# secondlaw-ai/skyrim

Hardware: AMD Instinct MI355X
Metric: 6-h forecast steps/sec on 721x1440 state, 1/2/4/8 MI355X; per-channel max rel-err vs ref (higher is better)
Workload: dtype f16; 1 GPU; Pangu 6-h autoregressive rollout, 721x1440x69 state (13 levels x 5 vars + 4 surface), random-init weights (64 M params), state resident in HBM, 1 ensemble membe; parallelism=single GPU, members=1, finite=True, rounding=compensated, term_plan=0x66f

## Files before the change

### skyrim_amd/csrc/api.hip

```cpp
#include <cstdio>
#include <cstdlib>
#include <cstring>
#include <string>
#include <type_traits>
#include <vector>

#include "../../include/skyrim_pangu.h"
#include "launchers.h"

using namespace skp;

namespace {

constexpr int kDepths[4] = {2, 6, 6, 2};
constexpr int kBiasRows = 3312;

int pad_to(int n, int mult, int* front, int pad_mode) {
    const int padded = (n + mult - 1) / mult * mult;
    if (front) *front = pad_mode == SKPANGU_PAD_CENTRE ? (padded - n) / 2 : 0;
    return padded;
}

bool make_geom(const skpangu_config& c, Geom& g) {
    if (c.n_lat < 8 || c.n_lon <= 0 || c.n_lon % 96 != 0) return false;
// ... 165 lines not shown
                                   : (qa_fused(1) ? kDepths[1] : 0) + (qa_fused(2) ? kDepths[2] : 0);
            if (nqa > 0) {
                const double qa_fl = fl[C_ATTN0 + o] + fl[C_QKV0 + o];
                const double qa_by = nt * C * 2 + mw * C * sa + 3 * C * C * wb + (double)g.types[r] * heads * 3456 * 2;
                fl[C_ATTN0 + o] = nqa == nblk ? qa_fl : (nqa * qa_fl + (nblk - nqa) * fl[C_ATTN0 + o]) / nblk;
                by[C_ATTN0 + o] = nqa == nblk ? qa_by : (nqa * qa_by + (nblk - nqa) * by[C_ATTN0 + o]) / nblk;
            }
            if (fused_block) {
                fl[C_FC1_0 + o] = 4 * nt * C * 4 * C;  by[C_FC1_0 + o] = 2 * nt * C * 4 + 8 * C * C * wb;
                fl[C_FC1_0 + o] += 2 * mw * C * C;     by[C_FC1_0 + o] += nt * C * sa + C * C * wb;
            }
        }
        fl[C_EMBED] = 2 * hw * 112 * 192 + 2 * 7 * hw * 160 * 192; by[C_EMBED] = (69.0 + 3) * g.n_lat * g.n_lon * 4 + g.ntok[0] * 192.0 * 4;
        fl[C_DOWN] = 2.0 * g.ntok[1] * 768 * 384;                   by[C_DOWN] = g.ntok[0] * 192.0 * 4 + g.ntok[1] * 384.0 * 4;
        fl[C_UP] = 2.0 * g.ntok[1] * 384 * 768 + 2.0 * g.ntok[0] * 192 * 192;
        by[C_UP] = g.ntok[1] * 384.0 * 4 + 2 * g.ntok[0] * 192.0 * sa + g.ntok[0] * 192.0 * 4;
        fl[C_RECOVER] = 2 * hw * 384 * 64 + 2 * 7 * hw * 384 * 160; by[C_RECOVER] = 2 * g.ntok[0] * 192.0 * 4 + 69.0 * g.n_lat * g.n_lon * 4;
        int k = 0;
        for (int c = 0; c < C_COUNT && k < cap; ++c, ++k) {
            std::memset(&out[k], 0, sizeof(out[k]));
            std::strncpy(out[k].name, names[c], sizeof(out[k].name) - 1);
            out[k].launches = cnt[c]; out[k].total_ms = ms[c]; out[k].flops = fl[c]; out[k].bytes = by[c];
        }
        *n = k;
        prof_used = 0;
        return hipSuccess;
    }

    LinW<T> take_lin(Arena& a, int N, int ldd) {
        LinW<T> l;
        const long long plane = (long long)N * ldd;
// ... 50 lines not shown
        Arena a{base, 0};
        const size_t n0 = (size_t)g.ntok[0] * 192, n1 = (size_t)g.ntok[1] * 384;
        wk.xs_plane[0] = (long long)n0; wk.xs_plane[1] = (long long)n1;
        wk.X1s = a.take<T>(n0 * 2); wk.X2s = a.take<T>(n1 * 2); wk.X4s = a.take<T>(n0 * 2);
        const size_t m0 = (size_t)g.mwin[0] * 192, m1 = (size_t)g.mwin[1] * 384;
        q_elems = m0 > m1 ? m0 : m1;
        wk.qkv_plane = (long long)q_elems;
        wk.q = a.take<f16>(q_elems); wk.k = a.take<f16>(q_elems); wk.vt = a.take<f16>(q_elems);
        ao_elems = q_elems;
        wk.ao_plane = (long long)ao_elems;
        wk.ao = a.take<T>(ao_elems * NPL);
        const size_t h0 = (size_t)g.ntok[0] * 768, h1 = (size_t)g.ntok[1] * 1536;
        hid_elems = h0 > h1 ? h0 : h1;
        wk.hid_plane = (long long)hid_elems;
        wk.hid = a.take<T>(hid_elems * NPL);
        wk.u_plane = (long long)n0;
        wk.u = a.take<T>(n0 * NPL);
        wk.stats = a.take<float2>((size_t)g.ntok[1]);
        ws_bytes = (a.off + 255) / 256 * 256;
    }

    explicit Engine(const Geom& geom, int qkv_a1 = 0, int mlp_mode = 0, int term_plan = 0) : g(geom) {
        fused_qa = getenv("SKP_SPLIT_ATTN") == nullptr;
        fused_block = mlp_mode == 0;
        rt_qkv = (std::is_same<P, PrecF16x3>::value && qkv_a1 && mlp_mode == 0);
        plan2 = (std::is_same<P, PrecF16x3>::value && fused_block) ? term_plan : 0;
        wk.qkv_a1 = qkv_a1;
        params = build_params(g, nullptr);
        plan_prepared(nullptr);
        plan_workspace(nullptr);
    }
    size_t prepared_bytes() const override { return prep_bytes; }
// ... 249 lines not shown
        for (int i = 0; i < kDepths[3]; ++i) CK(block_planes(3, i, wk.X4s, s));
        mark(C_RECOVER, s);
        CK((op_recover<P>(g, w, wk.X1s, wk.X4s, out, wk, s)));
        mark(-1, s);
        return hipSuccess;
    }
#undef CK

    bool debug(const std::string& n, void** p, size_t* bytes) override {
        auto set = [&](const void* ptr, size_t b) { *p = const_cast<void*>(ptr); *bytes = b; return true; };
        if (n == "q") return set(wk.q, q_elems * sizeof(f16));
        if (n == "k") return set(wk.k, q_elems * sizeof(f16));
        if (n == "vt") return set(wk.vt, q_elems * sizeof(f16));
        if (n == "ao") return set(wk.ao, ao_elems * NPL * sizeof(T));
        if (n == "hid") return set(wk.hid, hid_elems * NPL * sizeof(T));
        if (n == "u") return set(wk.u, (size_t)g.ntok[0] * 192 * NPL * sizeof(T));
        if (n == "x1") return set(wk.X1s, (size_t)g.ntok[0] * 192 * 2 * sizeof(T));
        if (n == "x2") return set(wk.X2s, (size_t)g.ntok[1] * 384 * 2 * sizeof(T));
        if (n == "x4") return set(wk.X4s, (size_t)g.ntok[0] * 192 * 2 * sizeof(T));
        if (n.rfind("widx", 0) == 0 && n.size() == 6) {
            const int r = n[4] - '0', roll = n[5] - '0';
            if (r < 0 || r > 1 || roll < 0 || roll > 1) return false;
            return set(w.widx[r][roll], (size_t)g.mwin[r] * 4);
        }
        if (n.rfind("bias_exp", 0) == 0) {
            const int b = atoi(n.c_str() + 8);
            if (b < 0 || b > 15) return false;
            return set(w.blk[b].bias_cmp, bias_elems[b] * sizeof(f16));
        }
        return false;
    }
// ... 147 lines not shown
```

### skyrim_amd/csrc/epilogues.h

```cpp
#pragma once
#include "common.h"

namespace skp {

__device__ __forceinline__ void pin(f32x4& v) { asm volatile("" : "+v"(v)); }

__device__ __forceinline__ void add8(f32x4& lo, f32x4& hi, const float4& b0, const float4& b1) {
    lo[0] += b0.x; lo[1] += b0.y; lo[2] += b0.z; lo[3] += b0.w;
    hi[0] += b1.x; hi[1] += b1.y; hi[2] += b1.z; hi[3] += b1.w;
}

constexpr int kEpiReduceBytes = 4096;
constexpr int kEpiTableBytes = 8192;
constexpr int kEpiScratch = kEpiReduceBytes + kEpiTableBytes;


template <class T>
struct EpStorePlanes {
    static constexpr bool kDualOrder = false;
    template <class TC> __device__ __forceinline__ void init(char*, int, int) const {}
    const float* bias;
    int ld, row_off;
    T* out;
    long long plane;
    template <class TC, bool SWAP>
    __device__ __forceinline__ void run(f32x4 (&acc)[TC::FM][TC::FN], int m0w, int n0w, int lane, int, int, char*, int M, int N, int) const {
        static_assert(SWAP && TC::FN % 2 == 0, "swapped order, fragment pairs");
        const int lm = lane & 15, l8 = (lane >> 4) * 8;
#pragma unroll
        for (int bp = 0; bp < TC::FN / 2; ++bp) {
            const int n = n0w + bp * 32 + l8;
            const float* bsrc = bias + (n < N ? n : 0);
            const float4 b0 = (bias != nullptr) ? *reinterpret_cast<const float4*>(bsrc) : make_float4(0.f, 0.f, 0.f, 0.f);
            const float4 b1 = (bias != nullptr) ? *reinterpret_cast<const float4*>(bsrc + 4) : make_float4(0.f, 0.f, 0.f, 0.f);
#pragma unroll
            for (int a = 0; a < TC::FM; ++a) { add8(acc[a][2 * bp], acc[a][2 * bp + 1], b0, b1); pin(acc[a][2 * bp]); pin(acc[a][2 * bp + 1]); }
        }
#pragma unroll
        for (int a = 0; a < TC::FM; ++a) {
            const int m = m0w + a * 16 + lm;
            if (m >= M) continue;
#pragma unroll
            for (int bp = 0; bp < TC::FN / 2; ++bp) {
                const int n = n0w + bp * 32 + l8;
                if (n >= N) continue;
                const f32x4 &x = acc[a][2 * bp], &y = acc[a][2 * bp + 1];
                const float vv[8] = {x[0], x[1], x[2], x[3], y[0], y[1], y[2], y[3]};
                store8_planes<T, 2>(out + blk_off(m + row_off, n, ld), plane, vv);
            }
        }
    }
};

template <class T, int NPL>
struct EpGelu {
    static constexpr bool kDualOrder = false;
    template <class TC> __device__ __forceinline__ void init(char*, int, int) const {}
    T* out;
    long long plane;
    const float* bias;
    int ld;
    template <class TC, bool SWAP>
    __device__ __forceinline__ void run(f32x4 (&acc)[TC::FM][TC::FN], int m0w, int n0w, int lane, int, int, char*, int M, int N, int) const {
        static_assert(SWAP && TC::FN % 2 == 0, "swapped order, fragment pairs");
        const int lm = lane & 15, l8 = (lane >> 4) * 8;
// ... 127 lines not shown
                            old.b.x + y[4], old.b.y + y[5], old.b.z + y[6], old.b.w + y[7]};
        store8_planes<T, 2>(xs + blk_off(row, c, ld), plane, v);
    }
};
template <class T, int NPL>
struct SinkStore {
    T* out;
    long long plane;
    static constexpr bool kLoads = false;
    __device__ __forceinline__ f32x8 load(long long, int, int) const { return f32x8{}; }
    __device__ __forceinline__ void put(long long row, int ld, int c, const float (&y)[8], const f32x8&) const {
        store8_planes<T, NPL>(out + blk_off(row, c, ld), plane, y);
    }
};

template <class RowMap, class Sink, int GROUP = 1>
struct EpLayerNorm {
    static constexpr bool kDualOrder = false;
    template <class TC> __device__ __forceinline__ void init(char* tab, int tid, int n0) const {
        float* t = reinterpret_cast<float*>(tab);
        for (int i = tid; i < TC::BN; i += TC::THREADS) {
            t[i] = gamma[i];
            t[TC::BN + i] = beta[i];
            t[2 * TC::BN + i] = bias != nullptr ? bias[n0 + i] : 0.f;
        }
    }
    RowMap map;
    Sink sink;
    const float* bias;
    const float* gamma;
    const float* beta;
    float eps;
    int n_groups = 0;
    template <class TC, bool SWAP>
    __device__ __forceinline__ void run(f32x4 (&acc)[TC::FM][TC::FN], int m0w, int n0w, int lane, int wm, int wn, char* smem, int M, int N, int ntile) const {
        static_assert(SWAP && TC::FN % 2 == 0, "swapped order, fragment pairs");
        static_assert(GROUP == 1 || (GROUP == TC::FM && !Sink::kLoads), "grouped rows: one member per fragment, no residual");
        constexpr int FM = TC::FM, FN = TC::FN, FP = TC::FN / 2, WN = TC::WN, BM = TC::BM, BN = TC::BN;
        const int l15 = lane & 15, l8 = (lane >> 4) * 8;
        const int nloc0 = n0w - ntile * BN;
        float* red = reinterpret_cast<float*>(smem);
        const float* tab = reinterpret_cast<const float*>(smem + kEpiReduceBytes);
        static_assert(3 * BN * 4 <= kEpiTableBytes && 2 * BM * WN * 4 <= kEpiReduceBytes, "epilogue LDS scratch");
#pragma unroll
        for (int bp = 0; bp < FP; ++bp) {
            const float* bsrc = tab + 2 * BN + nloc0 + bp * 32 + l8;
            const float4 b0 = *reinterpret_cast<const float4*>(bsrc), b1 = *reinterpret_cast<const float4*>(bsrc + 4);
#pragma unroll
            for (int a = 0; a < FM; ++a) add8(acc[a][2 * bp], acc[a][2 * bp + 1], b0, b1);
        }
        long long drow[FM];
        bool ok[FM];
#pragma unroll
        for (int a = 0; a < FM; ++a) {
            const int m = m0w + a * 16 + l15;
            const long long r = map.dest(m < M ? m : 0, ntile);
            ok[a] = m < M && r >= 0;
            drow[a] = ok[a] ? r : 0;
        }
        constexpr int PRE = FM < 3 ? FM : 3;
        f32x8 old[Sink::kLoads ? FM : 1][Sink::kLoads ? FP : 1];
        if constexpr (Sink::kLoads) {
#pragma unroll
            for (int a = 0; a < PRE; ++a)
#pragma unroll
                for (int bp = 0; bp < FP; ++bp) old[a][bp] = sink.load(drow[a], BN, nloc0 + bp * 32 + l8);
        }
        float mean[FM], rstd[FM];
#pragma unroll
        for (int a = 0; a < FM; ++a) {
            float s = 0.f;
#pragma unroll
            for (int b = 0; b < FN; ++b) s += (acc[a][b][0] + acc[a][b][1]) + (acc[a][b][2] + acc[a][b][3]);
            s += __shfl_xor(s, 16);
            s += __shfl_xor(s, 32);
            if (lane < 16) red[(wm * TC::WTM + a * 16 + lane) * WN + wn] = s;
        }
        __syncthreads();
#pragma unroll
        for (int a = 0; a < FM; ++a) {
            float s = 0.f;
#pragma unroll
            for (int w = 0; w < WN; ++w) s += red[(wm * TC::WTM + a * 16 + l15) * WN + w];
            mean[a] = s * (1.0f / BN);
        }
        float* red2 = red + BM * WN;
#pragma unroll
        for (int a = 0; a < FM; ++a) {
            float s = 0.f;
#pragma unroll
            for (int b = 0; b < FN; ++b) {
#pragma unroll
                for (int r = 0; r < 4; ++r) { const float d = acc[a][b][r] - mean[a]; s += d * d; }
            }
            s += __shfl_xor(s, 16);
            s += __shfl_xor(s, 32);
            if (lane < 16) red2[(wm * TC::WTM + a * 16 + lane) * WN + wn] = s;
        }
        __syncthreads();
#pragma unroll
        for (int a = 0; a < FM; ++a) {
            float s = 0.f;
#pragma unroll
            for (int w = 0; w < WN; ++w) s += red2[(wm * TC::WTM + a * 16 + l15) * WN + w];
            rstd[a] = rsqrtf(s * (1.0f / BN) + eps);
        }
        if constexpr (GROUP > 1) {
            const long long grow = (long long)(m0w / (16 * FM)) * 16 + l15;
#pragma unroll
            for (int bp = 0; bp < FP; ++bp) {
                const int c = nloc0 + bp * 32 + l8;
                const float4 g0 = *reinterpret_cast<const float4*>(tab + c), g1 = *reinterpret_cast<const float4*>(tab + c + 4);
                const float4 e0 = *reinterpret_cast<const float4*>(tab + BN + c), e1 = *reinterpret_cast<const float4*>(tab + BN + c + 4);
                float y[8] = {0.f, 0.f, 0.f, 0.f, 0.f, 0.f, 0.f, 0.f};
#pragma unroll
                for (int a = 0; a < FM; ++a) {
                    const f32x4 &x = acc[a][2 * bp], &z = acc[a][2 * bp + 1];
                    const float mu = mean[a], rs = rstd[a];
                    y[0] += (x[0] - mu) * rs * g0.x + e0.x; y[1] += (x[1] - mu) * rs * g0.y + e0.y;
                    y[2] += (x[2] - mu) * rs * g0.z + e0.z; y[3] += (x[3] - mu) * rs * g0.w + e0.w;
                    y[4] += (z[0] - mu) * rs * g1.x + e1.x; y[5] += (z[1] - mu) * rs * g1.y + e1.y;
                    y[6] += (z[2] - mu) * rs * g1.z + e1.z; y[7] += (z[3] - mu) * rs * g1.w + e1.w;
                }
                if (grow < n_groups) sink.put(grow, BN, c, y, old[0][0]);
            }
            return;
        }
#pragma unroll
        for (int a = 0; a < FM; ++a) {
#pragma unroll
            for (int bp = 0; bp < FP; ++bp) {
                const int c = nloc0 + bp * 32 + l8;
                const float4 g0 = *reinterpret_cast<const float4*>(tab + c), g1 = *reinterpret_cast<const float4*>(tab + c + 4);
                const float4 e0 = *reinterpret_cast<const float4*>(tab + BN + c), e1 = *reinterpret_cast<const float4*>(tab + BN + c + 4);
                const f32x4 &x = acc[a][2 * bp], &z = acc[a][2 * bp + 1];
                const float mu = mean[a], rs = rstd[a];
                const float y[8] = {(x[0] - mu) * rs * g0.x + e0.x, (x[1] - mu) * rs * g0.y + e0.y, (x[2] - mu) * rs * g0.z + e0.z, (x[3] - mu) * rs * g0.w + e0.w,
                                    (z[0] - mu) * rs * g1.x + e1.x, (z[1] - mu) * rs * g1.y + e1.y, (z[2] - mu) * rs * g1.z + e1.z, (z[3] - mu) * rs * g1.w + e1.w};
                if (ok[a]) sink.put(drow[a], BN, c, y, Sink::kLoads ? old[a][bp] : old[0][0]);
            }
            if constexpr (Sink::kLoads) {
                if (a + PRE < FM) {
#pragma unroll
                    for (int bp = 0; bp < FP; ++bp) old[a + PRE][bp] = sink.load(drow[a + PRE], BN, nloc0 + bp * 32 + l8);
                }
            }
        }
    }
};

struct EpRecover {
    static constexpr bool kDualOrder = false;
    template <class TC> __device__ __forceinline__ void init(char* tab, int tid, int) const {
// ... 47 lines not shown
```

### skyrim_amd/csrc/gemm.h

```cpp
#pragma once
#include "common.h"
#include "epilogues.h"

namespace skp {

template <int BM_, int BN_, int BK_, int WM_, int WN_>
struct TileCfg {
    static constexpr int BM = BM_, BN = BN_, BK = BK_, WM = WM_, WN = WN_;
    static constexpr int THREADS = 64 * WM * WN;
    static constexpr int WTM = BM / WM, WTN = BN / WN;
    static constexpr int FM = WTM / 16, FN = WTN / 16;
    static constexpr int CPR = BK / 8;
    static constexpr int A_CHUNKS = (BM * CPR + THREADS - 1) / THREADS;
    static constexpr int W_CHUNKS = (BN * CPR + THREADS - 1) / THREADS;
    static_assert(WTM % 16 == 0 && WTN % 16 == 0, "wave tile must be a multiple of 16x16");
    static_assert(THREADS % CPR == 0, "thread->slot mapping");
    static_assert(BK == 32 || BK == 64, "BK");
};

template <class P, class AL, class EP>
struct GemmArgs {
    AL al;
    EP ep;
    const typename P::T* W;
// ... 162 lines not shown

template <class P, class TC, class AL, class EP>
inline hipError_t launch_gemm(const GemmArgs<P, AL, EP>& g, hipStream_t stream) {
    dim3 grid((g.N + TC::BN - 1) / TC::BN, (g.M + TC::BM - 1) / TC::BM);
    if (grid.x == 0 || grid.y == 0) return hipSuccess;
    constexpr int smem = gemm_smem_bytes<P, TC>() + kEpiScratch;
    static_assert(smem <= 160 * 1024, "LDS per block");
    if (smem > 64 * 1024) {
        hipError_t e = hipFuncSetAttribute(reinterpret_cast<const void*>(gemm_kernel<P, TC, AL, EP>), hipFuncAttributeMaxDynamicSharedMemorySize, smem);
        if (e != hipSuccess) return e;
    }
    hipLaunchKernelGGL((gemm_kernel<P, TC, AL, EP>), grid, dim3(TC::THREADS), smem, stream, g);
    return hipGetLastError();
}

template <class TC, class AL, class EP>
hipError_t run_gemm(const AL& al, const EP& ep, const void* w, long long w_plane, int ldw, int M, int N, int K, hipStream_t s) {
    GemmArgs<PrecF16x3, AL, EP> g;
    g.al = al;
    g.ep = ep;
    g.W = static_cast<const f16*>(w);
    g.w_plane = w_plane;
    g.ldw = ldw;
    g.M = M; g.N = N; g.K = K;
    return launch_gemm<PrecF16x3, TC, AL, EP>(g, s);
}


}
```

### skyrim_amd/csrc/gemm_dma.h

```cpp
#pragma once
#include "gemm.h"

namespace skp {

typedef __attribute__((address_space(3))) void lds_void_t;
typedef const __attribute__((address_space(1))) void glb_void_t;

template <class T>
struct APlanes {
    const T* x;
    long long plane;
    int ld;
    const int* idx;
    int M;
    __device__ __forceinline__ void rows(int m, int k0, const T* zrow, const T*& hi, const T*& lo) const {
        int s = -1;
        if (m < M) s = idx ? idx[m] : m;
        if (s < 0) { hi = zrow; lo = zrow; return; }
        hi = x + blk_off(s, k0, ld);
        lo = hi + plane;
    }
    static constexpr int kSplitK = 0;
    __device__ __forceinline__ long long second_half_delta() const { return 0; }
};
// ... 72 lines not shown
            if constexpr (NA == 2) {
#pragma unroll
                for (int a = 0; a < FM; ++a)
                    acc[a][b] = SWAP ? OpT<T>::mfma(as_v8<T>(wf[0]), as_v8<T>(af[1][a]), acc[a][b])
                                     : OpT<T>::mfma(as_v8<T>(af[1][a]), as_v8<T>(wf[0]), acc[a][b]);
            }
#pragma unroll
            for (int a = 0; a < FM; ++a)
                acc[a][b] = SWAP ? OpT<T>::mfma(as_v8<T>(wf[0]), as_v8<T>(af[0][a]), acc[a][b])
                                 : OpT<T>::mfma(as_v8<T>(af[0][a]), as_v8<T>(wf[0]), acc[a][b]);
        }
    }
}

template <class P, class TC, class AS, class EP, bool SWAP>
__device__ __forceinline__ void gemm_dma_body(const DmaArgs<P, AS, EP>& g, char* smem, int m_tile, int n_tile) {
    typedef typename P::T T;
    constexpr int NA = P::NA, NW = P::NW, BM = TC::BM, BN = TC::BN, BK = TC::BK, CPR = TC::CPR;
    constexpr int RPI = 64 / CPR;
    constexpr int NWAVES = TC::THREADS / 64;
    constexpr int NI_A = NA * BM / RPI, NI_W = NW * BN / RPI, NI = NI_A + NI_W;
    constexpr int CNT = (NI + NWAVES - 1) / NWAVES;
    constexpr int STAGE = dma_stage_bytes<P, TC>();
    constexpr int A_BYTES = NA * BM * BK * 2;
    static_assert(BM % RPI == 0 && BN % RPI == 0, "tile rows per DMA instruction");

    const int tid = threadIdx.x, lane = tid & 63;
    const int wave = __builtin_amdgcn_readfirstlane(tid >> 6);
    const int wm = wave / TC::WN, wn = wave % TC::WN;
    const int m0 = m_tile * BM, n0 = n_tile * BN;

// ... 15 lines not shown
            dst_off[i] = (plane * BM + rb * RPI) * BK * 2;
            is_a[i] = true;
        } else if (q < NI) {
            const int qw = q - NI_A;
            const int plane = qw / (BN / RPI), rb = qw % (BN / RPI);
            const int r = rb * RPI + lr;
            const int chunk = (BK == 64) ? (lp ^ (r & 7)) : (lp ^ ((r >> 1) & 3));
            const int n = n0 + r;
            src[i] = n < g.N ? g.W + blk_off(n, chunk * 8, g.ldw) + plane * g.w_plane : g.zrow;
            dst_off[i] = A_BYTES + (plane * BN + rb * RPI) * BK * 2;
        }
    }
    const long long a_delta = g.as.second_half_delta();
    const int k_split = AS::kSplitK ? g.K / 2 : 0x7fffffff;

    f32x4 acc[TC::FM][TC::FN];
#pragma unroll
    for (int a = 0; a < TC::FM; ++a)
#pragma unroll
        for (int b = 0; b < TC::FN; ++b) acc[a][b] = f32x4{0.f, 0.f, 0.f, 0.f};

    const unsigned lds_base = (unsigned)(size_t)smem;
    auto issue = [&](int kt, int stage) {
        const int k = kt * BK;
#pragma unroll
        for (int i = 0; i < CNT; ++i) {
            if (wave + i * NWAVES < NI) {
                const T* p = src[i];
                const bool zero = (p == g.zrow);
                if (!zero) {
                    p += (long long)(k >> 5) * 512;
                    if (AS::kSplitK && is_a[i] && k >= k_split) p += a_delta;
                }
                glds16(p, lds_base + (unsigned)(stage * STAGE + dst_off[i]));
            }
        }
    };

    const int nk = g.K / BK;
    issue(0, 0);
    g.ep.template init<TC>(smem + 2 * STAGE + kEpiReduceBytes, tid, n0);
    for (int kt = 0; kt < nk; ++kt) {
        asm volatile("s_waitcnt vmcnt(0)" ::: "memory");
        __syncthreads();
        if (kt + 1 < nk) issue(kt + 1, (kt + 1) & 1);
        const char* st = smem + (kt & 1) * STAGE;
        mma_tile<P, TC, SWAP>(st, st + A_BYTES, acc, wm, wn, lane);
    }
    __syncthreads();
    g.ep.template run<TC, SWAP>(acc, m0 + wm * TC::WTM, n0 + wn * TC::WTN, lane, wm, wn, smem + 2 * STAGE, g.M, g.N, n_tile);
}

template <class P, class TC, class AS, class EP>
__global__ void __launch_bounds__(TC::THREADS) gemm_dma_kernel(const DmaArgs<P, AS, EP> g) {
    extern __shared__ __attribute__((aligned(16))) char smem[];
    const int nwg = gridDim.x, b = blockIdx.x;
    const int q = nwg >> 3, r = nwg & 7, xcd = b & 7;
    const int t = (xcd < r ? xcd * (q + 1) : r * (q + 1) + (xcd - r) * q) + (b >> 3);
    const int m_tile = t / g.nN, n_tile = t - m_tile * g.nN;
    if constexpr (EP::kDualOrder) {
        if (g.ep.unswapped(n_tile * TC::BN)) {
            gemm_dma_body<P, TC, AS, EP, false>(g, smem, m_tile, n_tile);
            return;
        }
    }
// ... 22 lines not shown
```

### skyrim_amd/csrc/launchers.h

```cpp
#pragma once
#include <hip/hip_runtime.h>
#include "common.h"

namespace skp {

struct Geom {
    int n_lat, n_lon, n_levels, n_channels, surf0;
    int lat_top;
    int Z, H1, W1, H2, W2;
    int Hp[2], top[2], nH[2], nW[2], types[2], nwin[2];
    int ntok[2], mwin[2];
    int roll_sign;
    float mask_value;
    int surface_last, qkv_order, bias_transposed;
};

template <class T>
struct LinW { const T* w; long long plane; int ldw; };

template <class T>
struct BlockW {
    LinW<T> qkv, proj, fc1, fc2;
    const T *w1f, *w2f;
    const T *projf, *qkvf;
// ... 14 lines not shown
    LinW<T> up1, up2;
    const float *up_g, *up_b;
    LinW<T> rec_u, rec_s;
    const float *rec_u_b, *rec_s_b;
    const int* widx[2][2];
    const int* winv[2][2];
};

template <class P>
struct Work {
    typedef typename P::T T;
    T *X1s, *X2s, *X4s;
    long long xs_plane[2];
    f16 *q, *k, *vt;
    long long qkv_plane;
    T *ao, *hid, *u;
    long long ao_plane, hid_plane, u_plane;
    const T* zrow;
    int qkv_a1;
    float2* stats;
};

template <class P>
struct AttnArgs {
    const f16 *q, *k, *vt;
    const f16* bias_cmp;
    typename P::T* out;
    long long out_plane;
    int ld_out, n_win, nW, heads;
    int out_planes = 0;
};

// ... 48 lines not shown
```

### skyrim_amd/csrc/ops_embed_recover.hip

```cpp
#include "tiles.h"

namespace skp {

template <class P>
hipError_t op_embed(const Geom& g, const ModelW<typename P::T>& w, const float* state, typename P::T* X1s, const Work<P>& wk, hipStream_t s) {
    typedef typename P::T T;
    typedef typename Tiles<P>::L192 TC;
    typedef EpStorePlanes<T> EP;
    const int hw = g.H1 * g.W1;
    {
        GemmArgs<P, ALIm2colSurface, EP> a;
        a.al = ALIm2colSurface{state, w.masks, w.mean, w.istd, g.n_lat, g.n_lon, g.lat_top, g.H1, g.W1, g.surf0, hw};
        a.ep = EP{w.embed_s_b, 192, 0, X1s, wk.xs_plane[0]};
        a.W = w.embed_s.w; a.w_plane = w.embed_s.plane; a.ldw = w.embed_s.ldw;
        a.M = hw; a.N = 192; a.K = 128;
        SKP_CHECK((launch_gemm<P, TC>(a, s)));
    }
    {
        GemmArgs<P, ALIm2colUpper, EP> a;
        a.al = ALIm2colUpper{state, w.mean, w.istd, g.n_lat, g.n_lon, g.lat_top, g.H1, g.W1, g.n_levels, (g.Z - 1) * hw};
        a.ep = EP{w.embed_u_b, 192, hw, X1s, wk.xs_plane[0]};
        a.W = w.embed_u.w; a.w_plane = w.embed_u.plane; a.ldw = w.embed_u.ldw;
        a.M = (g.Z - 1) * hw; a.N = 192; a.K = 160;
        SKP_CHECK((launch_gemm<P, TC>(a, s)));
    }
    return hipSuccess;
}

template <class P>
hipError_t op_recover(const Geom& g, const ModelW<typename P::T>& w, const typename P::T* skip_s, const typename P::T* x4_s, float* state,
                      const Work<P>& wk, hipStream_t s) {
    typedef typename P::T T;
    const int hw = g.H1 * g.W1;
    {
        DmaArgs<P, AConcatPlanes<T>, EpRecover> a;
        a.as = AConcatPlanes<T>{skip_s, x4_s, wk.xs_plane[0], 192, hw, 0};
        a.ep = EpRecover{state, w.rec_s_b, w.mean, w.std, g.n_lat, g.n_lon, g.lat_top, g.H1, g.W1, g.n_levels, 1, g.surf0};
        a.W = w.rec_s.w; a.w_plane = w.rec_s.plane; a.ldw = w.rec_s.ldw; a.zrow = wk.zrow;
        a.M = hw; a.N = 64; a.K = 384;
        SKP_CHECK((launch_gemm_dma<P, typename Tiles<P>::N64>(a, s)));
    }
// ... 18 lines not shown
```

### skyrim_amd/csrc/ops_updown.hip

```cpp
#include "tiles.h"

namespace skp {

template <class P>
hipError_t op_down(const Geom& g, const ModelW<typename P::T>& w, const typename P::T* X1s, typename P::T* X2s, const Work<P>& wk, hipStream_t s) {
    typedef typename P::T T;
    typedef EpStorePlanes<T> EP;
    SKP_CHECK((merge_stats<T>(X1s, wk.xs_plane[0], wk.stats, g.Z, g.H1, g.W1, g.H2, g.W2, 192, 1e-5f, s)));
    GemmArgs<P, ALMergeLN<T>, EP> a;
    a.al = ALMergeLN<T>{X1s, wk.xs_plane[0], wk.stats, w.down_g, w.down_b, g.H1, g.W1, g.H2, g.W2, 192, g.ntok[1]};
    a.ep = EP{nullptr, 384, 0, X2s, wk.xs_plane[1]};
    a.W = w.down.w; a.w_plane = w.down.plane; a.ldw = w.down.ldw;
    a.M = g.ntok[1]; a.N = 384; a.K = 768;
    return launch_gemm<P, typename Tiles<P>::D384>(a, s);
}

template <class P>
hipError_t op_up(const Geom& g, const ModelW<typename P::T>& w, const typename P::T* X2s, typename P::T* X4s, const Work<P>& wk, hipStream_t s) {
    typedef typename P::T T;
    typedef typename Tiles<P>::D192 TC;
    {
        typedef EpLayerNorm<RowMapPixelShuffle, SinkStore<T, P::NA>> EP;
        DmaArgs<P, APlanes<T>, EP> a;
        a.as = APlanes<T>{X2s, wk.xs_plane[1], 384, nullptr, g.ntok[1]};
        a.ep = EP{RowMapPixelShuffle{g.H1, g.W1, g.H2, g.W2}, SinkStore<T, P::NA>{wk.u, wk.u_plane}, nullptr, w.up_g, w.up_b, 1e-5f};
        a.W = w.up1.w; a.w_plane = w.up1.plane; a.ldw = w.up1.ldw; a.zrow = wk.zrow;
        a.M = g.ntok[1]; a.N = 768; a.K = 384;
        SKP_CHECK((launch_gemm_dma<P, TC>(a, s)));
    }
    {
        typedef EpStorePlanes<T> EP;
        DmaArgs<P, APlanes<T>, EP> a;
        a.as = APlanes<T>{wk.u, wk.u_plane, 192, nullptr, g.ntok[0]};
        a.ep = EP{nullptr, 192, 0, X4s, wk.xs_plane[0]};
        a.W = w.up2.w; a.w_plane = w.up2.plane; a.ldw = w.up2.ldw; a.zrow = wk.zrow;
        a.M = g.ntok[0]; a.N = 192; a.K = 192;
        SKP_CHECK((launch_gemm_dma<P, TC>(a, s)));
    }
    return hipSuccess;
}

template hipError_t op_down<PrecBF16x3>(const Geom&, const ModelW<bf16>&, const bf16*, bf16*, const Work<PrecBF16x3>&, hipStream_t);
template hipError_t op_down<PrecF16x3>(const Geom&, const ModelW<f16>&, const f16*, f16*, const Work<PrecF16x3>&, hipStream_t);
template hipError_t op_up<PrecBF16x3>(const Geom&, const ModelW<bf16>&, const bf16*, bf16*, const Work<PrecBF16x3>&, hipStream_t);
template hipError_t op_up<PrecF16x3>(const Geom&, const ModelW<f16>&, const f16*, f16*, const Work<PrecF16x3>&, hipStream_t);

}
```

Before: 73.71 steps/s.

## Fuse up-sample GEMM pair on-chip and merge embed GEMMs into one launch

The up-sampling path now runs its two GEMMs in one kernel. The layer-normed, pixel-shuffled output of the first GEMM is written into LDS and consumed directly by the second 192x192 GEMM, so the intermediate 'u' buffer and its HBM round trip go away. Separately, the surface and upper-air embed GEMMs are launched as one paired kernel split by blockIdx.y, saving a launch and a tail. The fused kernel uses a large LDS footprint (up to 160 KB), which lowers occupancy. It also runs the second GEMM serially in two halves per block, so parallelism may drop for this stage.

```diff
diff --git a/skyrim_amd/csrc/api.hip b/skyrim_amd/csrc/api.hip
--- a/skyrim_amd/csrc/api.hip
+++ b/skyrim_amd/csrc/api.hip
@@ -203,7 +203,7 @@
         fl[C_EMBED] = 2 * hw * 112 * 192 + 2 * 7 * hw * 160 * 192; by[C_EMBED] = (69.0 + 3) * g.n_lat * g.n_lon * 4 + g.ntok[0] * 192.0 * 4;
         fl[C_DOWN] = 2.0 * g.ntok[1] * 768 * 384;                   by[C_DOWN] = g.ntok[0] * 192.0 * 4 + g.ntok[1] * 384.0 * 4;
         fl[C_UP] = 2.0 * g.ntok[1] * 384 * 768 + 2.0 * g.ntok[0] * 192 * 192;
-        by[C_UP] = g.ntok[1] * 384.0 * 4 + 2 * g.ntok[0] * 192.0 * sa + g.ntok[0] * 192.0 * 4;
+        by[C_UP] = g.ntok[1] * 384.0 * 4 + g.ntok[0] * 192.0 * 4;
         fl[C_RECOVER] = 2 * hw * 384 * 64 + 2 * 7 * hw * 384 * 160; by[C_RECOVER] = 2 * g.ntok[0] * 192.0 * 4 + 69.0 * g.n_lat * g.n_lon * 4;
         int k = 0;
         for (int c = 0; c < C_COUNT && k < cap; ++c, ++k) {
@@ -284,8 +284,6 @@
         hid_elems = h0 > h1 ? h0 : h1;
         wk.hid_plane = (long long)hid_elems;
         wk.hid = a.take<T>(hid_elems * NPL);
-        wk.u_plane = (long long)n0;
-        wk.u = a.take<T>(n0 * NPL);
         wk.stats = a.take<float2>((size_t)g.ntok[1]);
         ws_bytes = (a.off + 255) / 256 * 256;
     }
@@ -565,7 +563,6 @@
         if (n == "vt") return set(wk.vt, q_elems * sizeof(f16));
         if (n == "ao") return set(wk.ao, ao_elems * NPL * sizeof(T));
         if (n == "hid") return set(wk.hid, hid_elems * NPL * sizeof(T));
-        if (n == "u") return set(wk.u, (size_t)g.ntok[0] * 192 * NPL * sizeof(T));
         if (n == "x1") return set(wk.X1s, (size_t)g.ntok[0] * 192 * 2 * sizeof(T));
         if (n == "x2") return set(wk.X2s, (size_t)g.ntok[1] * 384 * 2 * sizeof(T));
         if (n == "x4") return set(wk.X4s, (size_t)g.ntok[0] * 192 * 2 * sizeof(T));
diff --git a/skyrim_amd/csrc/epilogues.h b/skyrim_amd/csrc/epilogues.h
--- a/skyrim_amd/csrc/epilogues.h
+++ b/skyrim_amd/csrc/epilogues.h
@@ -14,6 +14,37 @@
 constexpr int kEpiTableBytes = 8192;
 constexpr int kEpiScratch = kEpiReduceBytes + kEpiTableBytes;
 
+
+template <class T, class TC, class Dest>
+__device__ __forceinline__ void store_planes_tile(f32x4 (&acc)[TC::FM][TC::FN], int m0w, int n0w, int lane, int M, int N, const float* bias,
+                                                  T* out, long long plane, int ld, const Dest& dest) {
+    static_assert(TC::FN % 2 == 0, "fragment pairs");
+    const int lm = lane & 15, l8 = (lane >> 4) * 8;
+#pragma unroll
+    for (int bp = 0; bp < TC::FN / 2; ++bp) {
+        const int n = n0w + bp * 32 + l8;
+        const float* bsrc = bias + (n < N ? n : 0);
+        const float4 b0 = (bias != nullptr) ? *reinterpret_cast<const float4*>(bsrc) : make_float4(0.f, 0.f, 0.f, 0.f);
+        const float4 b1 = (bias != nullptr) ? *reinterpret_cast<const float4*>(bsrc + 4) : make_float4(0.f, 0.f, 0.f, 0.f);
+#pragma unroll
+        for (int a = 0; a < TC::FM; ++a) { add8(acc[a][2 * bp], acc[a][2 * bp + 1], b0, b1); pin(acc[a][2 * bp]); pin(acc[a][2 * bp + 1]); }
+    }
+#pragma unroll
+    for (int a = 0; a < TC::FM; ++a) {
+        const int m = m0w + a * 16 + lm;
+        if (m >= M) continue;
+        const long long row = dest(m);
+        if (row < 0) continue;
+#pragma unroll
+        for (int bp = 0; bp < TC::FN / 2; ++bp) {
+            const int n = n0w + bp * 32 + l8;
+            if (n >= N) continue;
+            const f32x4 &x = acc[a][2 * bp], &y = acc[a][2 * bp + 1];
+            const float vv[8] = {x[0], x[1], x[2], x[3], y[0], y[1], y[2], y[3]};
+            store8_planes<T, 2>(out + blk_off(row, n, ld), plane, vv);
+        }
+    }
+}
 
 template <class T>
 struct EpStorePlanes {
@@ -25,30 +56,9 @@
     long long plane;
     template <class TC, bool SWAP>
     __device__ __forceinline__ void run(f32x4 (&acc)[TC::FM][TC::FN], int m0w, int n0w, int lane, int, int, char*, int M, int N, int) const {
-        static_assert(SWAP && TC::FN % 2 == 0, "swapped order, fragment pairs");
-        const int lm = lane & 15, l8 = (lane >> 4) * 8;
-#pragma unroll
-        for (int bp = 0; bp < TC::FN / 2; ++bp) {
-            const int n = n0w + bp * 32 + l8;
-            const float* bsrc = bias + (n < N ? n : 0);
-            const float4 b0 = (bias != nullptr) ? *reinterpret_cast<const float4*>(bsrc) : make_float4(0.f, 0.f, 0.f, 0.f);
-            const float4 b1 = (bias != nullptr) ? *reinterpret_cast<const float4*>(bsrc + 4) : make_float4(0.f, 0.f, 0.f, 0.f);
-#pragma unroll
-            for (int a = 0; a < TC::FM; ++a) { add8(acc[a][2 * bp], acc[a][2 * bp + 1], b0, b1); pin(acc[a][2 * bp]); pin(acc[a][2 * bp + 1]); }
-        }
-#pragma unroll
-        for (int a = 0; a < TC::FM; ++a) {
-            const int m = m0w + a * 16 + lm;
-            if (m >= M) continue;
-#pragma unroll
-            for (int bp = 0; bp < TC::FN / 2; ++bp) {
-                const int n = n0w + bp * 32 + l8;
-                if (n >= N) continue;
-                const f32x4 &x = acc[a][2 * bp], &y = acc[a][2 * bp + 1];
-                const float vv[8] = {x[0], x[1], x[2], x[3], y[0], y[1], y[2], y[3]};
-                store8_planes<T, 2>(out + blk_off(m + row_off, n, ld), plane, vv);
-            }
-        }
+        static_assert(SWAP, "swapped order");
+        const int off = row_off;
+        store_planes_tile<T, TC>(acc, m0w, n0w, lane, M, N, bias, out, plane, ld, [off](int m) { return (long long)(m + off); });
     }
 };
 
@@ -206,6 +216,56 @@
     }
 };
 
+template <class TC>
+__device__ __forceinline__ void ln_row_stats(const f32x4 (&acc)[TC::FM][TC::FN], int lane, int wm, int wn, float* red, float eps,
+                                             float (&mean)[TC::FM], float (&rstd)[TC::FM]) {
+    constexpr int FM = TC::FM, FN = TC::FN, WN = TC::WN, BM = TC::BM, BN = TC::BN;
+    const int l15 = lane & 15;
+#pragma unroll
+    for (int a = 0; a < FM; ++a) {
+        float s = 0.f;
+#pragma unroll
+        for (int b = 0; b < FN; ++b) s += (acc[a][b][0] + acc[a][b][1]) + (acc[a][b][2] + acc[a][b][3]);
+        s += __shfl_xor(s, 16);
+        s += __shfl_xor(s, 32);
+        if (lane < 16) red[(wm * TC::WTM + a * 16 + lane) * WN + wn] = s;
+    }
+    __syncthreads();
+#pragma unroll
+    for (int a = 0; a < FM; ++a) {
+        float s = 0.f;
+#pragma unroll
+        for (int w = 0; w < WN; ++w) s += red[(wm * TC::WTM + a * 16 + l15) * WN + w];
+        mean[a] = s * (1.0f / BN);
+    }
+    float* red2 = red + BM * WN;
+#pragma unroll
+    for (int a = 0; a < FM; ++a) {
+        float s = 0.f;
+#pragma unroll
+        for (int b = 0; b < FN; ++b) {
+#pragma unroll
+            for (int r = 0; r < 4; ++r) { const float d = acc[a][b][r] - mean[a]; s += d * d; }
+        }
+        s += __shfl_xor(s, 16);
+        s += __shfl_xor(s, 32);
+        if (lane < 16) red2[(wm * TC::WTM + a * 16 + lane) * WN + wn] = s;
+    }
+    __syncthreads();
+#pragma unroll
+    for (int a = 0; a < FM; ++a) {
+        float s = 0.f;
+#pragma unroll
+        for (int w = 0; w < WN; ++w) s += red2[(wm * TC::WTM + a * 16 + l15) * WN + w];
+        rstd[a] = rsqrtf(s * (1.0f / BN) + eps);
+    }
+}
+__device__ __forceinline__ void ln_affine8(const f32x4& x, const f32x4& z, float mu, float rs, const float4& g0, const float4& g1,
+                                           const float4& e0, const float4& e1, float (&y)[8]) {
+    y[0] = (x[0] - mu) * rs * g0.x + e0.x; y[1] = (x[1] - mu) * rs * g0.y + e0.y; y[2] = (x[2] - mu) * rs * g0.z + e0.z; y[3] = (x[3] - mu) * rs * g0.w + e0.w;
+    y[4] = (z[0] - mu) * rs * g1.x + e1.x; y[5] = (z[1] - mu) * rs * g1.y + e1.y; y[6] = (z[2] - mu) * rs * g1.z + e1.z; y[7] = (z[3] - mu) * rs * g1.w + e1.w;
+}
+
 template <class RowMap, class Sink, int GROUP = 1>
 struct EpLayerNorm {
     static constexpr bool kDualOrder = false;
@@ -228,7 +288,7 @@
     __device__ __forceinline__ void run(f32x4 (&acc)[TC::FM][TC::FN], int m0w, int n0w, int lane, int wm, int wn, char* smem, int M, int N, int ntile) const {
         static_assert(SWAP && TC::FN % 2 == 0, "swapped order, fragment pairs");
         static_assert(GROUP == 1 || (GROUP == TC::FM && !Sink::kLoads), "grouped rows: one member per fragment, no residual");
-        constexpr int FM = TC::FM, FN = TC::FN, FP = TC::FN / 2, WN = TC::WN, BM = TC::BM, BN = TC::BN;
+        constexpr int FM = TC::FM, FP = TC::FN / 2, WN = TC::WN, BM = TC::BM, BN = TC::BN;
         const int l15 = lane & 15, l8 = (lane >> 4) * 8;
         const int nloc0 = n0w - ntile * BN;
         float* red = reinterpret_cast<float*>(smem);
@@ -259,44 +319,7 @@
                 for (int bp = 0; bp < FP; ++bp) old[a][bp] = sink.load(drow[a], BN, nloc0 + bp * 32 + l8);
         }
         float mean[FM], rstd[FM];
-#pragma unroll
-        for (int a = 0; a < FM; ++a) {
-            float s = 0.f;
-#pragma unroll
-            for (int b = 0; b < FN; ++b) s += (acc[a][b][0] + acc[a][b][1]) + (acc[a][b][2] + acc[a][b][3]);
-            s += __shfl_xor(s, 16);
-            s += __shfl_xor(s, 32);
-            if (lane < 16) red[(wm * TC::WTM + a * 16 + lane) * WN + wn] = s;
-        }
-        __syncthreads();
-#pragma unroll
-        for (int a = 0; a < FM; ++a) {
-            float s = 0.f;
-#pragma unroll
-            for (int w = 0; w < WN; ++w) s += red[(wm * TC::WTM + a * 16 + l15) * WN + w];
-            mean[a] = s * (1.0f / BN);
-        }
-        float* red2 = red + BM * WN;
-#pragma unroll
-        for (int a = 0; a < FM; ++a) {
-            float s = 0.f;
-#pragma unroll
-            for (int b = 0; b < FN; ++b) {
-#pragma unroll
-                for (int r = 0; r < 4; ++r) { const float d = acc[a][b][r] - mean[a]; s += d * d; }
-            }
-            s += __shfl_xor(s, 16);
-            s += __shfl_xor(s, 32);
-            if (lane < 16) red2[(wm * TC::WTM + a * 16 + lane) * WN + wn] = s;
-        }
-        __syncthreads();
-#pragma unroll
-        for (int a = 0; a < FM; ++a) {
-            float s = 0.f;
-#pragma unroll
-            for (int w = 0; w < WN; ++w) s += red2[(wm * TC::WTM + a * 16 + l15) * WN + w];
-            rstd[a] = rsqrtf(s * (1.0f / BN) + eps);
-        }
+        ln_row_stats<TC>(acc, lane, wm, wn, red, eps, mean, rstd);
         if constexpr (GROUP > 1) {
             const long long grow = (long long)(m0w / (16 * FM)) * 16 + l15;
 #pragma unroll
@@ -327,8 +350,8 @@
                 const float4 e0 = *reinterpret_cast<const float4*>(tab + BN + c), e1 = *reinterpret_cast<const float4*>(tab + BN + c + 4);
                 const f32x4 &x = acc[a][2 * bp], &z = acc[a][2 * bp + 1];
                 const float mu = mean[a], rs = rstd[a];
-                const float y[8] = {(x[0] - mu) * rs * g0.x + e0.x, (x[1] - mu) * rs * g0.y + e0.y, (x[2] - mu) * rs * g0.z + e0.z, (x[3] - mu) * rs * g0.w + e0.w,
-                                    (z[0] - mu) * rs * g1.x + e1.x, (z[1] - mu) * rs * g1.y + e1.y, (z[2] - mu) * rs * g1.z + e1.z, (z[3] - mu) * rs * g1.w + e1.w};
+                float y[8];
+                ln_affine8(x, z, mu, rs, g0, g1, e0, e1, y);
                 if (ok[a]) sink.put(drow[a], BN, c, y, Sink::kLoads ? old[a][bp] : old[0][0]);
             }
             if constexpr (Sink::kLoads) {
diff --git a/skyrim_amd/csrc/gemm.h b/skyrim_amd/csrc/gemm.h
--- a/skyrim_amd/csrc/gemm.h
+++ b/skyrim_amd/csrc/gemm.h
@@ -200,6 +200,25 @@
     return hipGetLastError();
 }
 
+template <class P, class TC, class AL0, class AL1, class EP>
+__global__ void __launch_bounds__(TC::THREADS) gemm_pair_kernel(const GemmArgs<P, AL0, EP> g0, const GemmArgs<P, AL1, EP> g1, const int ny0) {
+    extern __shared__ __attribute__((aligned(16))) char smem[];
+    static_assert(!EP::kDualOrder, "swapped order only");
+    if ((int)blockIdx.y < ny0) gemm_body<P, TC, AL0, EP, true>(g0, smem, blockIdx.x, blockIdx.y);
+    else gemm_body<P, TC, AL1, EP, true>(g1, smem, blockIdx.x, blockIdx.y - ny0);
+}
+
+template <class P, class TC, class AL0, class AL1, class EP>
+inline hipError_t launch_gemm_pair(const GemmArgs<P, AL0, EP>& g0, const GemmArgs<P, AL1, EP>& g1, hipStream_t stream) {
+    const int nx = (g0.N + TC::BN - 1) / TC::BN, ny0 = (g0.M + TC::BM - 1) / TC::BM, ny1 = (g1.M + TC::BM - 1) / TC::BM;
+    if ((g1.N + TC::BN - 1) / TC::BN != nx) return hipErrorInvalidValue;
+    if (nx == 0 || ny0 + ny1 == 0) return hipSuccess;
+    constexpr int smem = gemm_smem_bytes<P, TC>() + kEpiScratch;
+    static_assert(smem <= 64 * 1024, "LDS per block");
+    hipLaunchKernelGGL((gemm_pair_kernel<P, TC, AL0, AL1, EP>), dim3(nx, ny0 + ny1), dim3(TC::THREADS), smem, stream, g0, g1, ny0);
+    return hipGetLastError();
+}
+
 template <class TC, class AL, class EP>
 hipError_t run_gemm(const AL& al, const EP& ep, const void* w, long long w_plane, int ldw, int M, int N, int K, hipStream_t s) {
     GemmArgs<PrecF16x3, AL, EP> g;
diff --git a/skyrim_amd/csrc/gemm_dma.h b/skyrim_amd/csrc/gemm_dma.h
--- a/skyrim_amd/csrc/gemm_dma.h
+++ b/skyrim_amd/csrc/gemm_dma.h
@@ -110,7 +110,8 @@
 }
 
 template <class P, class TC, class AS, class EP, bool SWAP>
-__device__ __forceinline__ void gemm_dma_body(const DmaArgs<P, AS, EP>& g, char* smem, int m_tile, int n_tile) {
+__device__ __forceinline__ void gemm_dma_mainloop(const DmaArgs<P, AS, EP>& g, char* smem, char* epi, int m_tile, int n_tile,
+                                                  f32x4 (&acc)[TC::FM][TC::FN]) {
     typedef typename P::T T;
     constexpr int NA = P::NA, NW = P::NW, BM = TC::BM, BN = TC::BN, BK = TC::BK, CPR = TC::CPR;
     constexpr int RPI = 64 / CPR;
@@ -156,7 +157,6 @@
     const long long a_delta = g.as.second_half_delta();
     const int k_split = AS::kSplitK ? g.K / 2 : 0x7fffffff;
 
-    f32x4 acc[TC::FM][TC::FN];
 #pragma unroll
     for (int a = 0; a < TC::FM; ++a)
 #pragma unroll
@@ -181,7 +181,7 @@
 
     const int nk = g.K / BK;
     issue(0, 0);
-    g.ep.template init<TC>(smem + 2 * STAGE + kEpiReduceBytes, tid, n0);
+    g.ep.template init<TC>(epi + kEpiReduceBytes, tid, n0);
     for (int kt = 0; kt < nk; ++kt) {
         asm volatile("s_waitcnt vmcnt(0)" ::: "memory");
         __syncthreads();
@@ -189,8 +189,17 @@
         const char* st = smem + (kt & 1) * STAGE;
         mma_tile<P, TC, SWAP>(st, st + A_BYTES, acc, wm, wn, lane);
     }
+}
+
+template <class P, class TC, class AS, class EP, bool SWAP>
+__device__ __forceinline__ void gemm_dma_body(const DmaArgs<P, AS, EP>& g, char* smem, int m_tile, int n_tile) {
+    constexpr int STAGE = dma_stage_bytes<P, TC>();
+    const int lane = threadIdx.x & 63, wave = __builtin_amdgcn_readfirstlane(threadIdx.x >> 6);
+    const int wm = wave / TC::WN, wn = wave % TC::WN;
+    f32x4 acc[TC::FM][TC::FN];
+    gemm_dma_mainloop<P, TC, AS, EP, SWAP>(g, smem, smem + 2 * STAGE, m_tile, n_tile, acc);
     __syncthreads();
-    g.ep.template run<TC, SWAP>(acc, m0 + wm * TC::WTM, n0 + wn * TC::WTN, lane, wm, wn, smem + 2 * STAGE, g.M, g.N, n_tile);
+    g.ep.template run<TC, SWAP>(acc, m_tile * TC::BM + wm * TC::WTM, n_tile * TC::BN + wn * TC::WTN, lane, wm, wn, smem + 2 * STAGE, g.M, g.N, n_tile);
 }
 
 template <class P, class TC, class AS, class EP>
diff --git a/skyrim_amd/csrc/launchers.h b/skyrim_amd/csrc/launchers.h
--- a/skyrim_amd/csrc/launchers.h
+++ b/skyrim_amd/csrc/launchers.h
@@ -52,8 +52,8 @@
     long long xs_plane[2];
     f16 *q, *k, *vt;
     long long qkv_plane;
-    T *ao, *hid, *u;
-    long long ao_plane, hid_plane, u_plane;
+    T *ao, *hid;
+    long long ao_plane, hid_plane;
     const T* zrow;
     int qkv_a1;
     float2* stats;
diff --git a/skyrim_amd/csrc/ops_embed_recover.hip b/skyrim_amd/csrc/ops_embed_recover.hip
--- a/skyrim_amd/csrc/ops_embed_recover.hip
+++ b/skyrim_amd/csrc/ops_embed_recover.hip
@@ -8,23 +8,17 @@
     typedef typename Tiles<P>::L192 TC;
     typedef EpStorePlanes<T> EP;
     const int hw = g.H1 * g.W1;
-    {
-        GemmArgs<P, ALIm2colSurface, EP> a;
-        a.al = ALIm2colSurface{state, w.masks, w.mean, w.istd, g.n_lat, g.n_lon, g.lat_top, g.H1, g.W1, g.surf0, hw};
-        a.ep = EP{w.embed_s_b, 192, 0, X1s, wk.xs_plane[0]};
-        a.W = w.embed_s.w; a.w_plane = w.embed_s.plane; a.ldw = w.embed_s.ldw;
-        a.M = hw; a.N = 192; a.K = 128;
-        SKP_CHECK((launch_gemm<P, TC>(a, s)));
-    }
-    {
-        GemmArgs<P, ALIm2colUpper, EP> a;
-        a.al = ALIm2colUpper{state, w.mean, w.istd, g.n_lat, g.n_lon, g.lat_top, g.H1, g.W1, g.n_levels, (g.Z - 1) * hw};
-        a.ep = EP{w.embed_u_b, 192, hw, X1s, wk.xs_plane[0]};
-        a.W = w.embed_u.w; a.w_plane = w.embed_u.plane; a.ldw = w.embed_u.ldw;
-        a.M = (g.Z - 1) * hw; a.N = 192; a.K = 160;
-        SKP_CHECK((launch_gemm<P, TC>(a, s)));
-    }
-    return hipSuccess;
+    GemmArgs<P, ALIm2colSurface, EP> a;
+    a.al = ALIm2colSurface{state, w.masks, w.mean, w.istd, g.n_lat, g.n_lon, g.lat_top, g.H1, g.W1, g.surf0, hw};
+    a.ep = EP{w.embed_s_b, 192, 0, X1s, wk.xs_plane[0]};
+    a.W = w.embed_s.w; a.w_plane = w.embed_s.plane; a.ldw = w.embed_s.ldw;
+    a.M = hw; a.N = 192; a.K = 128;
+    GemmArgs<P, ALIm2colUpper, EP> b;
+    b.al = ALIm2colUpper{state, w.mean, w.istd, g.n_lat, g.n_lon, g.lat_top, g.H1, g.W1, g.n_levels, (g.Z - 1) * hw};
+    b.ep = EP{w.embed_u_b, 192, hw, X1s, wk.xs_plane[0]};
+    b.W = w.embed_u.w; b.w_plane = w.embed_u.plane; b.ldw = w.embed_u.ldw;
+    b.M = (g.Z - 1) * hw; b.N = 192; b.K = 160;
+    return launch_gemm_pair<P, TC>(a, b, s);
 }
 
 template <class P>
diff --git a/skyrim_amd/csrc/ops_updown.hip b/skyrim_amd/csrc/ops_updown.hip
--- a/skyrim_amd/csrc/ops_updown.hip
+++ b/skyrim_amd/csrc/ops_updown.hip
@@ -15,29 +15,146 @@
     return launch_gemm<P, typename Tiles<P>::D384>(a, s);
 }
 
+struct SinkOnChip {};
+template <class P>
+struct UpFusedArgs {
+    typedef typename P::T T;
+    typedef EpLayerNorm<RowMapPixelShuffle, SinkOnChip> EP1;
+    DmaArgs<P, APlanes<T>, EP1> g1;
+    const T* W2;
+    long long w2_plane;
+    int ldw2;
+    T* out;
+    long long out_plane;
+};
+
+template <class P>
+struct UpFusedCfg {
+    typedef typename Tiles<P>::D192 TC;
+    typedef TileCfg<128, 192, TC::BK, 4, 2> TC2;
+    static constexpr int KSTEPS2 = 192 / TC::BK;
+    static constexpr int A2_KSTEP = P::NA * TC2::BM * TC::BK * 2;
+    static constexpr int A2_BYTES = KSTEPS2 * A2_KSTEP;
+    static constexpr int W2_STAGE = P::NW * 192 * TC::BK * 2;
+    static constexpr int EPI = A2_BYTES + 2 * W2_STAGE;
+    static constexpr int SMEM = EPI + kEpiScratch;
+    static_assert(P::NA == 2 && P::NW == 2 && TC::BK == 32 && TC::BN == 192 && TC::WM == 4 && TC::WN == 2, "three-term plane modes");
+    static_assert(EPI >= 2 * dma_stage_bytes<P, TC>() && SMEM <= 160 * 1024, "LDS plan");
+};
+
+template <class P>
+__global__ void __launch_bounds__(UpFusedCfg<P>::TC::THREADS) up_fused_kernel(const UpFusedArgs<P> u) {
+    typedef typename P::T T;
+    typedef UpFusedCfg<P> CF;
+    typedef typename CF::TC TC;
+    typedef typename CF::TC2 TC2;
+    constexpr int BK = TC::BK, FM = TC::FM, FP = TC::FN / 2, BN = TC::BN;
+    extern __shared__ __attribute__((aligned(16))) char smem[];
+    const int nwg = gridDim.x, b = blockIdx.x;
+    const int q8 = nwg >> 3, r8 = nwg & 7, xcd = b & 7;
+    const int t = (xcd < r8 ? xcd * (q8 + 1) : r8 * (q8 + 1) + (xcd - r8) * q8) + (b >> 3);
+    const int m_tile = t / u.g1.nN, n_tile = t - m_tile * u.g1.nN;
+    const int tid = threadIdx.x, lane = tid & 63;
+    const int wave = __builtin_amdgcn_readfirstlane(tid >> 6);
+    const int wm = wave / TC::WN, wn = wave % TC::WN;
+    const int l15 = lane & 15, l8 = (lane >> 4) * 8;
+
+    f32x4 acc[TC::FM][TC::FN];
+    gemm_dma_mainloop<P, TC, APlanes<T>, typename UpFusedArgs<P>::EP1, true>(u.g1, smem, smem + CF::EPI, m_tile, n_tile, acc);
+    __syncthreads();
+
+    constexpr int NI_W = P::NW * 192 / 16, CNT = NI_W / 8;
+    static_assert(NI_W % 8 == 0, "DMA instructions per wave");
+    const T* wsrc[CNT];
+    int wdst[CNT];
+#pragma unroll
+    for (int i = 0; i < CNT; ++i) {
+        const int q = wave + i * 8;
+        const int plane = q / 12, rb = q % 12;
+        const int r = rb * 16 + lane / 4;
+        const int chunk = (lane % 4) ^ ((r >> 1) & 3);
+        wsrc[i] = u.W2 + blk_off(r, chunk * 8, u.ldw2) + plane * u.w2_plane;
+        wdst[i] = CF::A2_BYTES + (plane * 192 + rb * 16) * BK * 2;
+    }
+    const unsigned lds_base = (unsigned)(size_t)smem;
+    auto issue_w = [&](int kt, int stage) {
+#pragma unroll
+        for (int i = 0; i < CNT; ++i) glds16(wsrc[i] + (long long)kt * 512, lds_base + (unsigned)(stage * CF::W2_STAGE + wdst[i]));
+    };
+    issue_w(0, 0);
+
+    float* red = reinterpret_cast<float*>(smem + CF::EPI);
+    const float* tab = reinterpret_cast<const float*>(smem + CF::EPI + kEpiReduceBytes);
+    const int nloc0 = wn * TC::WTN;
+#pragma unroll
+    for (int bp = 0; bp < FP; ++bp) {
+        const float* bsrc = tab + 2 * BN + nloc0 + bp * 32 + l8;
+        const float4 b0 = *reinterpret_cast<const float4*>(bsrc), b1 = *reinterpret_cast<const float4*>(bsrc + 4);
+#pragma unroll
+        for (int a = 0; a < FM; ++a) add8(acc[a][2 * bp], acc[a][2 * bp + 1], b0, b1);
+    }
+    float mean[FM], rstd[FM];
+    ln_row_stats<TC>(acc, lane, wm, wn, red, u.g1.ep.eps, mean, rstd);
+
+    const RowMapPixelShuffle map = u.g1.ep.map;
+#pragma unroll
+    for (int half = 0; half < 2; ++half) {
+        if ((wm >> 1) == half) {
+#pragma unroll
+            for (int a = 0; a < FM; ++a) {
+                const int rloc = (wm & 1) * TC::WTM + a * 16 + l15;
+#pragma unroll
+                for (int bp = 0; bp < FP; ++bp) {
+                    const int c = nloc0 + bp * 32 + l8;
+                    const float4 g0 = *reinterpret_cast<const float4*>(tab + c), g1 = *reinterpret_cast<const float4*>(tab + c + 4);
+                    const float4 e0 = *reinterpret_cast<const float4*>(tab + BN + c), e1 = *reinterpret_cast<const float4*>(tab + BN + c + 4);
+                    float y[8];
+                    ln_affine8(acc[a][2 * bp], acc[a][2 * bp + 1], mean[a], rstd[a], g0, g1, e0, e1, y);
+                    uint4 o[P::NA];
+                    split8<T, P::NA>(y, o);
+                    char* dst = smem + (c >> 5) * CF::A2_KSTEP + lds_off<BK>(rloc, lane >> 4);
+#pragma unroll
+                    for (int p = 0; p < P::NA; ++p) *reinterpret_cast<uint4*>(dst + p * (TC2::BM * BK * 2)) = o[p];
+                }
+            }
+        }
+        f32x4 acc2[TC2::FM][TC2::FN];
+#pragma unroll
+        for (int a = 0; a < TC2::FM; ++a)
+#pragma unroll
+            for (int bb = 0; bb < TC2::FN; ++bb) acc2[a][bb] = f32x4{0.f, 0.f, 0.f, 0.f};
+        for (int kt = 0; kt < CF::KSTEPS2; ++kt) {
+            asm volatile("s_waitcnt vmcnt(0)" ::: "memory");
+            __syncthreads();
+            if (kt + 1 < CF::KSTEPS2) issue_w(kt + 1, (kt + 1) & 1);
+            mma_tile<P, TC2, true>(smem + kt * CF::A2_KSTEP, smem + CF::A2_BYTES + (kt & 1) * CF::W2_STAGE, acc2, wm, wn, lane);
+        }
+        if (half == 0) {
+            __syncthreads();
+            issue_w(0, 0);
+        }
+        store_planes_tile<T, TC2>(acc2, m_tile * TC::BM + half * TC2::BM + wm * TC2::WTM, wn * TC2::WTN, lane, u.g1.M, 192, nullptr, u.out,
+                                  u.out_plane, 192, [&](int m) { return map.dest(m, n_tile); });
+    }
+}
+
 template <class P>
 hipError_t op_up(const Geom& g, const ModelW<typename P::T>& w, const typename P::T* X2s, typename P::T* X4s, const Work<P>& wk, hipStream_t s) {
     typedef typename P::T T;
-    typedef typename Tiles<P>::D192 TC;
-    {
-        typedef EpLayerNorm<RowMapPixelShuffle, SinkStore<T, P::NA>> EP;
-        DmaArgs<P, APlanes<T>, EP> a;
-        a.as = APlanes<T>{X2s, wk.xs_plane[1], 384, nullptr, g.ntok[1]};
-        a.ep = EP{RowMapPixelShuffle{g.H1, g.W1, g.H2, g.W2}, SinkStore<T, P::NA>{wk.u, wk.u_plane}, nullptr, w.up_g, w.up_b, 1e-5f};
-        a.W = w.up1.w; a.w_plane = w.up1.plane; a.ldw = w.up1.ldw; a.zrow = wk.zrow;
-        a.M = g.ntok[1]; a.N = 768; a.K = 384;
-        SKP_CHECK((launch_gemm_dma<P, TC>(a, s)));
-    }
-    {
-        typedef EpStorePlanes<T> EP;
-        DmaArgs<P, APlanes<T>, EP> a;
-        a.as = APlanes<T>{wk.u, wk.u_plane, 192, nullptr, g.ntok[0]};
-        a.ep = EP{nullptr, 192, 0, X4s, wk.xs_plane[0]};
-        a.W = w.up2.w; a.w_plane = w.up2.plane; a.ldw = w.up2.ldw; a.zrow = wk.zrow;
-        a.M = g.ntok[0]; a.N = 192; a.K = 192;
-        SKP_CHECK((launch_gemm_dma<P, TC>(a, s)));
-    }
-    return hipSuccess;
+    typedef UpFusedCfg<P> CF;
+    UpFusedArgs<P> u;
+    u.g1.as = APlanes<T>{X2s, wk.xs_plane[1], 384, nullptr, g.ntok[1]};
+    u.g1.ep = typename UpFusedArgs<P>::EP1{RowMapPixelShuffle{g.H1, g.W1, g.H2, g.W2}, SinkOnChip{}, nullptr, w.up_g, w.up_b, 1e-5f};
+    u.g1.W = w.up1.w; u.g1.w_plane = w.up1.plane; u.g1.ldw = w.up1.ldw; u.g1.zrow = wk.zrow;
+    u.g1.M = g.ntok[1]; u.g1.N = 768; u.g1.K = 384;
+    u.g1.nM = (u.g1.M + CF::TC::BM - 1) / CF::TC::BM; u.g1.nN = 768 / CF::TC::BN;
+    u.W2 = w.up2.w; u.w2_plane = w.up2.plane; u.ldw2 = w.up2.ldw;
+    u.out = X4s; u.out_plane = wk.xs_plane[0];
+    if (u.g1.nM == 0) return hipSuccess;
+    if (w.up2.ldw != 192) return hipErrorInvalidValue;
+    SKP_CHECK(hipFuncSetAttribute(reinterpret_cast<const void*>(up_fused_kernel<P>), hipFuncAttributeMaxDynamicSharedMemorySize, CF::SMEM));
+    hipLaunchKernelGGL((up_fused_kernel<P>), dim3((unsigned)(u.g1.nM * u.g1.nN)), dim3(CF::TC::THREADS), CF::SMEM, s, u);
+    return hipGetLastError();
 }
 
 template hipError_t op_down<PrecBF16x3>(const Geom&, const ModelW<bf16>&, const bf16*, bf16*, const Work<PrecBF16x3>&, hipStream_t);
```

New measurement: 74.15 steps/s (median of 6 runs). No clear change (+0.6%).
